# tzmhuang/OmniIsaacGymEnvs

Measured on AMD Instinct MI355X. Metric: env-steps/s (physics+obs+reward) Humanoid 4096 envs @1/2/4/8 MI355X, higher is better.
Workload: dtype f32

## Files before the change

include/mi_geom.h:

```cpp
#ifndef MI_GEOM_H
#define MI_GEOM_H

#include <math.h>

#if defined(__HIPCC__)
#define MI_GEOM_FN static inline __host__ __device__
#else
#define MI_GEOM_FN static inline
#endif

#if defined(__clang__)
#define MI_GEOM_NO_CONTRACT _Pragma("clang fp contract(off)")
#else
#define MI_GEOM_NO_CONTRACT
#endif

MI_GEOM_FN float mi_g_clamp01(float x) { return x < 0.0f ? 0.0f : (x > 1.0f ? 1.0f : x); }

MI_GEOM_FN void mi_segment_closest(const float* a0, const float* a1, const float* b0,
                                   const float* b1, float* ca, float* cb) {
    MI_GEOM_NO_CONTRACT
    float d1[3], d2[3], r[3];
    for (int k = 0; k < 3; ++k) { d1[k] = a1[k] - a0[k]; d2[k] = b1[k] - b0[k]; r[k] = a0[k] - b0[k]; }
    const float a = d1[0] * d1[0] + d1[1] * d1[1] + d1[2] * d1[2];
    const float e = d2[0] * d2[0] + d2[1] * d2[1] + d2[2] * d2[2];
    const float f = d2[0] * r[0] + d2[1] * r[1] + d2[2] * r[2];
    float s = 0.0f, t = 0.0f;
    if (a <= 1e-12f && e <= 1e-12f) {
        s = 0.0f; t = 0.0f;
    } else if (a <= 1e-12f) {
        s = 0.0f; t = mi_g_clamp01(f / e);
    } else {
        const float c = d1[0] * r[0] + d1[1] * r[1] + d1[2] * r[2];
        if (e <= 1e-12f) {
            t = 0.0f; s = mi_g_clamp01(-c / a);
        } else {
            const float b = d1[0] * d2[0] + d1[1] * d2[1] + d1[2] * d2[2];
            const float den = a * e - b * b;
            s = den > 1e-12f ? mi_g_clamp01((b * f - c * e) / den) : 0.0f;
            t = (b * s + f) / e;
            if (t < 0.0f) { t = 0.0f; s = mi_g_clamp01(-c / a); }
            else if (t > 1.0f) { t = 1.0f; s = mi_g_clamp01((b - c) / a); }
        }
    }
    for (int k = 0; k < 3; ++k) { ca[k] = a0[k] + d1[k] * s; cb[k] = b0[k] + d2[k] * t; }
}

MI_GEOM_FN void mi_contact_basis(const float* n, float* t1, float* t2) {
    MI_GEOM_NO_CONTRACT
    const float ax[3] = {n[0] < 0.57735f && n[0] > -0.57735f ? 1.0f : 0.0f,
                         n[0] < 0.57735f && n[0] > -0.57735f ? 0.0f : 1.0f, 0.0f};
    float c[3] = {n[1] * ax[2] - n[2] * ax[1], n[2] * ax[0] - n[0] * ax[2], n[0] * ax[1] - n[1] * ax[0]};
    const float cl = sqrtf(c[0] * c[0] + c[1] * c[1] + c[2] * c[2]);
    for (int k = 0; k < 3; ++k) t1[k] = c[k] / cl;
    t2[0] = n[1] * t1[2] - n[2] * t1[1];
    t2[1] = n[2] * t1[0] - n[0] * t1[2];
    t2[2] = n[0] * t1[1] - n[1] * t1[0];
}

MI_GEOM_FN float mi_pair_contact(const float* a0, const float* a1, float ra, const float* b0,
                                 const float* b1, float rb, float* pc, float* n) {
    MI_GEOM_NO_CONTRACT
    float ca[3], cb[3];
    mi_segment_closest(a0, a1, b0, b1, ca, cb);
    float d[3] = {ca[0] - cb[0], ca[1] - cb[1], ca[2] - cb[2]};
    const float dist = sqrtf(d[0] * d[0] + d[1] * d[1] + d[2] * d[2]);
    if (dist > 1e-9f) {
        for (int k = 0; k < 3; ++k) n[k] = d[k] / dist;
    } else {
        n[0] = 0.0f; n[1] = 0.0f; n[2] = 1.0f;
    }
    const float gap = dist - ra - rb;
    for (int k = 0; k < 3; ++k) pc[k] = cb[k] + n[k] * (rb + 0.5f * gap);
    return gap;
}

#endif
```

include/mi_sim.h:

```cpp
#ifndef MI_SIM_H
#define MI_SIM_H

#include <stdint.h>

#ifdef __cplusplus
extern "C" {
#endif

#define MI_ABI_VERSION 4

enum {
    MI_OK = 0,
    MI_E_NULL = -1,
    MI_E_SHAPE = -2,
    MI_E_HIP = -3,
    MI_E_MODEL = -4,
    MI_E_ARG = -5,
    MI_E_NODEV = -6,
    MI_E_STATE = -7
};

enum { MI_TASK_CARTPOLE = 0, MI_TASK_ANT = 1, MI_TASK_HUMANOID = 2 };

enum {
// ... 128 lines not shown
int mi_get_state_mirror(mi_sim* sim, void* stream);

int mi_sim_step(mi_sim* sim, int32_t substeps, void* stream);
int mi_sim_flush(mi_sim* sim, void* stream);

int mi_task_configure(mi_sim* sim, const mi_task_params* tp);
int mi_task_pre_step(mi_sim* sim, const float* actions , int64_t* reset_buf,
                     int64_t* progress_buf, float* potentials, float* prev_potentials,
                     float* actions_out , void* stream);
int mi_task_reset_idx(mi_sim* sim, const int64_t* env_ids, int32_t n, int64_t* reset_buf,
                      int64_t* progress_buf, float* potentials, float* prev_potentials,
                      void* stream);
int mi_task_post_step(mi_sim* sim, const float* actions , float* obs ,
                      float* rew , int64_t* reset_buf, int64_t* progress_buf,
                      float* potentials, float* prev_potentials, void* stream);
int mi_task_post_kernel(const mi_sim* sim, int32_t* kernel, int32_t* grid);
int mi_task_observations(mi_sim* sim, const float* actions , float* obs ,
                         float* potentials, float* prev_potentials, void* stream);
int mi_task_metrics(mi_sim* sim, const float* actions, const float* obs, float* rew,
                    const float* potentials, const float* prev_potentials, void* stream);
int mi_task_is_done(mi_sim* sim, const float* obs, int64_t* reset_buf, const int64_t* progress_buf,
                    void* stream);
int mi_env_step(mi_sim* sim, const float* actions , int32_t substeps,
                float* obs_out , float* obs_task ,
                float* rew , int64_t* reset_buf, int64_t* progress_buf,
                float* potentials, float* prev_potentials, float* actions_out ,
                float* rew_out , int64_t* reset_out , void* stream);
int mi_sim_time_launches(mi_sim* sim, int32_t every, int32_t capacity);
int mi_sim_launch_times(mi_sim* sim, float* ms_out, int32_t max_out, int32_t* n_out);

enum { MI_DR_OP_ADDITIVE = 0, MI_DR_OP_SCALING = 1 };
enum { MI_DR_DIST_GAUSSIAN = 0, MI_DR_DIST_UNIFORM = 1, MI_DR_DIST_LOGUNIFORM = 2 };
typedef struct mi_dr_noise {
    int32_t enabled;
    int32_t operation;
    int32_t distribution;
    int32_t frequency_interval;
    float params[2];
} mi_dr_noise;
typedef struct mi_dr_params {
    mi_dr_noise obs_on_reset, obs_on_interval, act_on_reset, act_on_interval;
} mi_dr_params;
int mi_task_set_dr(mi_sim* sim, const mi_dr_params* dr );
int mi_dr_apply_actions(mi_sim* sim, float* actions , const int64_t* reset_buf, void* stream);
int mi_dr_apply_observations(mi_sim* sim, float* obs , const int64_t* reset_buf,
                             void* stream);
int mi_get_dr_state(mi_sim* sim, uint32_t* out );

enum { MI_ENVP_GRAVITY = 0,
       MI_ENVP_FRICTION = 1,
       MI_ENVP_DAMPING = 2,
       MI_ENVP_ARMATURE = 3    };
int mi_set_env_params(mi_sim* sim, int32_t attr, const float* values ,
                      const int64_t* idx , int32_t n, void* stream);
int mi_get_env_params(mi_sim* sim, int32_t attr, float* out , void* stream);
int mi_sim_clear_env_params(mi_sim* sim);

enum { MI_DR_OP_DIRECT = 2 };
typedef struct mi_dr_phys_sched {
    int32_t enabled;
    int32_t operation;
    int32_t distribution;
    int32_t frequency_interval;
    const float* p0;
    const float* p1;
} mi_dr_phys_sched;
typedef struct mi_dr_phys_params {
    mi_dr_phys_sched on_reset[4], on_interval[4];
    int32_t min_frequency;
} mi_dr_phys_params;
int mi_sim_set_phys_dr(mi_sim* sim, const mi_dr_phys_params* dr );
int mi_dr_phys_step(mi_sim* sim, const int64_t* reset_buf , void* stream);
int mi_get_phys_dr_state(mi_sim* sim, uint32_t* out );

int mi_fill_uniform(mi_sim* sim, float* out , int32_t cols, uint64_t seed,
                    uint64_t step, float lo, float hi, void* stream);
int mi_get_reset_count(mi_sim* sim, uint32_t* out );
int mi_set_reset_count(mi_sim* sim, const uint32_t* in );
int mi_sim_pair_load(mi_sim* sim, int32_t* out , const int32_t* in ,
                     int32_t pairing);
int mi_sim_nan_count(mi_sim* sim, int64_t* count);
int mi_sim_kernel_path(const mi_sim* sim, int32_t* path, int32_t* topology, int32_t* lds_bytes);
int mi_sim_w_rows_lds(const mi_sim* sim, int32_t* rows);
int mi_abi_version(void);
const char* mi_build_id(void);
const char* mi_last_error(void);

#ifdef __cplusplus
}
#endif
#endif
```

omniisaacgymenvs_amd/csrc/mi_pair.hpp:

```cpp
#pragma once
#include "mi_wave.hpp"

#ifndef MI_PAIR_SOLVE_PD
#define MI_PAIR_SOLVE_PD 3
#endif
#ifndef MI_PRIO_C1
#define MI_PRIO_C1 12
#endif
#ifndef MI_PRIO_C2
#define MI_PRIO_C2 18
#endif
#ifndef MI_PRIO_C3
#define MI_PRIO_C3 27
#endif

namespace mi {

MI_D float pbc(float v, int k) {
    const float a = readlane(v, k), b = readlane(v, k + 32);
    return (pair_l64() & 32) ? b : a;
}
template <int K>
MI_D float pbcc(float v) {
    static_assert(K >= 0 && K < 32, "lane of the half");
// ... 200 lines not shown
    wave_sync();
    STAMP(0);
    for (int l = 1 + lane; l < L; l += 32) wave_link_local(mc, t, sm, l);
    wave_sync();
    for (int l = lane; l < L; l += 32) wave_link_forward<TP::kEnvP>(mc, nr, t, sm, l, p, ep);
    wave_sync();
    STAMP(1);
    float* aux = sm + t.s_X;
    {
        const pv4* recs = reinterpret_cast<const pv4*>(sm + t.s_F);
        for (int l = lane; l < L; l += 32) {
            pv4 a0 = recs[4 * l], a1 = recs[4 * l + 1], a2 = recs[4 * l + 2], a3 = recs[4 * l + 3];
            for (int di = mc.desc_start(l); di < mc.desc_start(l + 1); ++di) {
                const int d = mc.desc(di);
                a0 += recs[4 * d];
                a1 += recs[4 * d + 1];
                a2 += recs[4 * d + 2];
                a3 += recs[4 * d + 3];
            }
            pv4* o = reinterpret_cast<pv4*>(aux) + 4 * l;
            o[0] = a0; o[1] = a1; o[2] = a2; o[3] = a3;
        }
    }
    wave_sync();
    STAMP(2);
    phase_p3_bias_crba<Grp32, TP>(lane, i, D, nv, nr, dt, us, rhs, Mx, Ss, mc, t, st, aux, ep);
    wave_sync();
    STAMP(3);
    float Mc[TP::nvc];
    ct_load_columns<TP>(Mx, lane, Mc);
    const float dvec = ct_ltdl_pair<TP>(lane, Mc);
    STAMP(5);
    {
        const int dj = lane < nr ? lane : __builtin_popcount(mc.mask(lane < nv ? lane - nr + 1 : 0)) - 1;
        ct_publish_factor<TP>(lane, dj, Mc, dvec, sm + t.s_L);
    }
    STAMP(4);
    int ncon = 0;
    {
        const float rpz = sm[t.s_rp + 2];
        for (int c0 = 0; c0 < t.npts; c0 += 32) {
            const int c = c0 + lane;
            bool act = false;
            float pc[3] = {0, 0, 0}, bn = 0.0f;
            int l = 0;
            if (c < t.npts) {
                l = (int)mc.pf(MP_LINK, c);
                const float pl[3] = {mc.pf(MP_X, c), mc.pf(MP_X + 1, c), mc.pf(MP_X + 2, c)};
                float R[9], x[3];
#pragma unroll
                for (int q = 0; q < 9; ++q) R[q] = sm[t.s_R + 9 * l + q];
                m3_vec(R, pl, x);
#pragma unroll
                for (int q = 0; q < 3; ++q) x[q] += sm[t.s_o + 3 * l + q];
                const float rr = mc.pf(MP_RAD, c);
                const float gap = rpz + x[2] - rr;
                act = gap < p.contact_offset;
                pc[0] = x[0]; pc[1] = x[1]; pc[2] = x[2] - rr;
                const float d = gap - p.rest_offset;
                bn = p.tgs ? d : row_bias(p, d, dt, true);
            }
            const unsigned mask = hballot(act);
            if (act) {
                const int ci = ncon + __popc(mask & lanemask_lt(lane));
#pragma unroll
                for (int q = 0; q < 3; ++q) sm[t.s_cp + 3 * ci + q] = pc[q];
                sm[t.s_cl + ci] = (float)l;
                sm[t.s_cl2 + ci] = -1.0f;
#pragma unroll
                for (int tt = 0; tt < 3; ++tt) {
                    const int r = 3 * ci + tt;
                    sm[t.s_rl + r] = (float)l;
                    sm[t.s_rb + r] = tt == 0 ? bn : 0.0f;
                }
            }
            ncon += __popc(mask);
        }
    }
    if constexpr (TP::kSelf) {
        if (t.self_on) {
            float* seg = sm + t.s_seg;
            float* bnd = seg + 8 * t.ngeoms;
            const float* geo = mcb + t.mc_geo;
            const int2* gpr = reinterpret_cast<const int2*>(t.g_pairs);
            int2 gpf[5];
#pragma unroll
            for (int q = 0; q < 5; ++q) {
                const int pi = 32 * q + lane;
                gpf[q] = pi < t.npairs ? gpr[pi] : make_int2(0, 0);
            }
            for (int g = lane; g < t.ngeoms; g += 32) {
                const float* A = geo + 8 * g;
                const int l = (int)A[0];
                float R[9], a0[3], a1[3];
#pragma unroll
                for (int q = 0; q < 9; ++q) R[q] = sm[t.s_R + 9 * l + q];
                m3_vec(R, A + 1, a0); m3_vec(R, A + 4, a1);
#pragma unroll
                for (int q = 0; q < 3; ++q) {
                    seg[8 * g + q] = a0[q] + sm[t.s_o + 3 * l + q];
                    seg[8 * g + 3 + q] = a1[q] + sm[t.s_o + 3 * l + q];
                }
                seg[8 * g + 6] = A[7];
                seg[8 * g + 7] = (float)l;
                float e2 = 0.0f;
#pragma unroll
                for (int q = 0; q < 3; ++q) {
                    bnd[4 * g + q] = sm[t.s_o + 3 * l + q] + 0.5f * (a0[q] + a1[q]);
                    e2 += (a1[q] - a0[q]) * (a1[q] - a0[q]);
                }
                bnd[4 * g + 3] = 0.5f * sqrtf(e2) + A[7];
            }
            wave_sync();
            int* surv = reinterpret_cast<int*>(sm + t.s_surv);
            int nsv = 0;
            const float slack = p.contact_offset + 1e-3f;
            auto broad = [&](int pb, int2 gpq, bool pref) {
                const int pi = pb + lane;
                bool keep = false;
                int2 gp = make_int2(0, 0);
                if (pi < t.npairs) {
                    gp = pref ? gpq : gpr[pi];
                    const float4 A = *reinterpret_cast<const float4*>(bnd + 4 * gp.x);
                    const float4 B = *reinterpret_cast<const float4*>(bnd + 4 * gp.y);
                    const float cx = A.x - B.x, cy = A.y - B.y, cz = A.z - B.z;
                    const float reach = A.w + B.w + slack;
                    keep = cx * cx + cy * cy + cz * cz < reach * reach;
                }
                const unsigned mask = hballot(keep);
                if (keep) surv[nsv + __popc(mask & lanemask_lt(lane))] = gp.x | (gp.y << 16);
                nsv += __popc(mask);
            };
            sfor<0, 5>([&](auto Q) { if (32 * (int)Q < t.npairs) broad(32 * (int)Q, gpf[Q], true); });
            for (int pb = 160; pb < t.npairs; pb += 32) broad(pb, make_int2(0, 0), false);
            wave_sync();
            int budget = (MI_MAX_ROWS - 3 * ncon - t.nlimc) / 3;
            const int nsv_max = pmax(nsv);
            for (int sb = 0; sb < nsv_max; sb += 32) {
                const int sidx = sb + lane;
                bool act = false;
                float pc[3], n[3], bn = 0.0f;
                int la = 0, lb = 0;
                if (sidx < nsv && budget > 0) {
                    const int pk = surv[sidx];
                    const float* A = seg + 8 * (pk & 0xffff);
                    const float* B = seg + 8 * (pk >> 16);
                    la = (int)A[7]; lb = (int)B[7];
                    const float gap = mi_pair_contact(A, A + 3, A[6], B, B + 3, B[6], pc, n);
                    act = gap < p.contact_offset;
                    const float d = gap - p.rest_offset;
                    bn = p.tgs ? d : row_bias(p, d, dt, true);
                }
                const unsigned mask = hballot(act);
                const int rank = __popc(mask & lanemask_lt(lane));
                if (act && rank < budget) {
                    const int ci = ncon + rank;
#pragma unroll
                    for (int q = 0; q < 3; ++q) { sm[t.s_cp + 3 * ci + q] = pc[q]; sm[t.s_cn + 3 * ci + q] = n[q]; }
                    sm[t.s_cl + ci] = (float)la;
                    sm[t.s_cl2 + ci] = (float)lb;
#pragma unroll
                    for (int tt = 0; tt < 3; ++tt) {
                        const int r = 3 * ci + tt;
                        sm[t.s_rl + r] = (float)la;
                        sm[t.s_rb + r] = tt == 0 ? bn : 0.0f;
                    }
                }
                const int took = budget > 0 ? min(__popc(mask), budget) : 0;
                ncon += took;
                budget -= took;
            }
        }
    }
    const int nc = 3 * ncon;
    {
        const int cr = pmax(nc);
        if (cr > MI_PRIO_C3 && prio < 3) { __builtin_amdgcn_s_setprio(3); prio = 3; }
        else if (cr > MI_PRIO_C2 && prio < 2) { __builtin_amdgcn_s_setprio(2); prio = 2; }
        else if (cr > MI_PRIO_C1 && prio < 1) { __builtin_amdgcn_s_setprio(1); prio = 1; }
    }
    wave_sync();
    STAMP(6);
    constexpr bool kSpec = TP::D >= MI_PAIR_LIM_SPEC_MIN_D;
    unsigned cmask = 0u, nmask = 0u;
    if constexpr (kSpec) {
        bool cand = false, near = false;
        if (lane < D) {
            const float lo = mc.lf(MC_LO, lane + 1), hi = mc.lf(MC_HI, lane + 1);
            const float qj = sm[t.s_q + lane], qp = qj + dt * us[nr + lane];
            const float mg = MI_PAIR_LIM_NEAR;
            cand = lo < hi;
            near = cand && (qj < lo + mg || qp < lo + mg || qj > hi - mg || qp > hi - mg);
        }
        cmask = hballot(cand);
        nmask = hballot(near);
    }
    const unsigned fmask = cmask & ~nmask;
    const int nN = __popc(nmask);
    const int nspec = kSpec ? min(__popc(cmask), 31 - (nc & 31)) : t.nlimc;
    int total = nc + 1 + nspec;
    int total_max = pmax(total);
    unsigned rem = 0u;
    int nrows = nc;
    unsigned limact = 0u;
    auto limit_rows = [&](const auto& res, bool here, bool rhs_lane) {
        constexpr int NR = sizeof(res) / sizeof(res[0]);
        if (rhs_lane) {
#pragma unroll
            for (int c = 0; c < NR; ++c)
                if (c < TP::nv) us[c] = us[c] + dt * res[c];
        }
        wave_sync();
        bool act = false;
        float bl = 0.0f, sg = 0.0f;
        if (here && lane < D) {
            const int l = lane + 1, k = nr + lane;
            const float lo = mc.lf(MC_LO, l), hi = mc.lf(MC_HI, l);
            if (lo < hi) {
                const float qj = sm[t.s_q + lane];
                const float qp = qj + dt * us[k];
                float d = 0.0f;
                if (qj < lo || qp < lo) { d = qj - lo; sg = 1.0f; act = true; }
                else if (qj > hi || qp > hi) { d = hi - qj; sg = -1.0f; act = true; }
                bl = p.tgs ? d : row_bias(p, d, dt, true);
            }
        }
        const unsigned lb = hballot(act);
        if (here) limact = lb;
        if (act) {
            const int rl = nc + __popc(limact & lanemask_lt(lane));
// ... 795 lines not shown
```

omniisaacgymenvs_amd/csrc/mi_sim.hip:

```cpp
#include <hip/hip_runtime.h>
#include <hip/hip_ext.h>

#include <cmath>
#include <cstdarg>
#include <cstdio>
#include <cstring>
#include <string>
#include <vector>
#include <algorithm>

#include "mi_artic.hpp"
#include "mi_device.hpp"
#include "mi_task.hpp"
#include "mi_wave.hpp"
#include "mi_pair.hpp"
#include "mi_link.hpp"
#include "mi_dyn.hpp"
#include "mi_msolve.hpp"
#include "mi_idyn.hpp"

using namespace mi;

static thread_local std::string g_err;

// ... 1143 lines not shown
    if (s->wave) {
        const char* tsel = getenv("MI_SIM_TOPO");
        s->topo = (tsel && std::string(tsel) == "runtime") ? 0 : match_topology(cx.md, self_on);
    }
    return MI_OK;
}

static int create_tree_tables(mi_sim* s, CreateCtx& cx) {
    const mi_model_desc* md = cx.md;
    const DevModel& m = s->dm;
    WaveTabs& t = s->wt;
    const int L = m.L;
    const std::vector<int>& dof_parent = cx.dof_parent;
    std::vector<int> depth(L, 0);
    int maxd = 0;
    for (int l = 1; l < L; ++l) { depth[l] = depth[md->parent[l]] + 1; maxd = std::max(maxd, depth[l]); }
    t.nlev = maxd + 1;
    std::vector<int> lev_start(t.nlev + 1, 0), lev_links;
    for (int d = 0; d < t.nlev; ++d) {
        lev_start[d] = (int)lev_links.size();
        for (int l = 0; l < L; ++l) if (depth[l] == d) lev_links.push_back(l);
    }
    lev_start[t.nlev] = (int)lev_links.size();
    std::vector<int> child_start(L + 1, 0), child_list;
    for (int l = 0; l < L; ++l) {
        child_start[l] = (int)child_list.size();
        for (int c = l + 1; c < L; ++c) if (md->parent[c] == l) child_list.push_back(c);
    }
    child_start[L] = (int)child_list.size();
    std::vector<int>&desc_start = cx.desc_start, &desc_list = cx.desc_list;
    desc_start.assign(L + 1, 0);
    for (int l = 0; l < L; ++l) {
        desc_start[l] = (int)desc_list.size();
        for (int c = l + 1; c < L; ++c) {
            int x = md->parent[c];
            while (x > l) x = md->parent[x];
            if (x == l) desc_list.push_back(c);
        }
    }
    desc_start[L] = (int)desc_list.size();
    if (desc_list.empty()) desc_list.push_back(0);
    std::vector<int>& anc_start = cx.anc_start;
    anc_start.assign(m.nv + 1, 0);
    std::vector<int> anc_list;
    int na_max = 0;
    for (int k = 0; k < m.nv; ++k) {
        anc_start[k] = (int)anc_list.size();
        for (int j = dof_parent[k]; j >= 0; j = dof_parent[j]) anc_list.push_back(j);
        na_max = std::max(na_max, (int)anc_list.size() - anc_start[k]);
    }
    anc_start[m.nv] = (int)anc_list.size();
    std::vector<unsigned long long>& link_mask = cx.link_mask;
    link_mask.assign(L, 0ull);
    for (int l = 0; l < L; ++l) {
        unsigned long long msk = 0ull;
        for (int k = 0; k < m.nr; ++k) msk |= 1ull << k;
        for (int x = l; x > 0; x = md->parent[x]) msk |= 1ull << (m.nr + x - 1);
        link_mask[l] = msk;
    }
    std::vector<unsigned char> tri_p, tri_q;
    for (int q = 0; q < na_max; ++q)
        for (int p2 = 0; p2 <= q; ++p2) { tri_p.push_back((unsigned char)p2); tri_q.push_back((unsigned char)q); }
    if (tri_p.empty()) { tri_p.push_back(0); tri_q.push_back(0); }
    if (child_list.empty()) child_list.push_back(0);
    if (anc_list.empty()) anc_list.push_back(0);
    UPW(lev_start, lev_start); UPW(lev_links, lev_links); UPW(child_start, child_start);
    UPW(child_list, child_list); UPW(anc_start, anc_start); UPW(anc_list, anc_list);
    UPW(desc_start, desc_start); UPW(desc_list, desc_list);
    std::vector<int>&chain_start = cx.chain_start, &chain_list = cx.chain_list;
    chain_start.assign(L + 1, 0);
    for (int l = 0; l < L; ++l) {
        chain_start[l] = (int)chain_list.size();
        std::vector<int> up;
        for (int x = l; x > 0; x = md->parent[x]) up.push_back(x);
        chain_list.insert(chain_list.end(), up.rbegin(), up.rend());
    }
    chain_start[L] = (int)chain_list.size();
    if (chain_list.empty()) chain_list.push_back(0);
    UPW(chain_start, chain_start); UPW(chain_list, chain_list);
    UPW(link_mask, link_mask); UPW(tri_p, tri_p); UPW(tri_q, tri_q);
    return MI_OK;
}

static int create_constant_block(mi_sim* s, const CreateCtx& cx) {
    const mi_model_desc* md = cx.md;
    WaveTabs& t = s->wt;
    const int L = s->dm.L;
    const bool self_on = cx.self_on;
    const std::vector<int>&pt_geom = cx.pt_geom, &pt_end = cx.pt_end, &chain_start = cx.chain_start,
                          &chain_list = cx.chain_list, &desc_start = cx.desc_start, &desc_list = cx.desc_list;
    const std::vector<unsigned long long>& link_mask = cx.link_mask;
    {
        const int np = (int)pt_geom.size(), ns = md->num_sensors;
        std::vector<float> mcb((size_t)MC_NLINKF * L, 0.0f);
        for (int l = 0; l < L; ++l) {
            auto put = [&](int f, float v) { mcb[(size_t)f * L + l] = v; };
            for (int c = 0; c < 3; ++c) {
                put(MC_POS + c, md->pos[3 * l + c]); put(MC_AXIS + c, md->axis[3 * l + c]);
                put(MC_COM + c, md->com[3 * l + c]);
            }
            for (int c = 0; c < 4; ++c) put(MC_QUAT + c, md->quat[4 * l + c]);
            for (int c = 0; c < 6; ++c) put(MC_INER + c, md->inertia[6 * l + c]);
            put(MC_JTYPE, (float)md->jtype[l]); put(MC_MASS, md->mass[l]);
            put(MC_ARM, md->armature[l]); put(MC_DAMP, md->damping[l]);
            put(MC_LO, md->lower[l]); put(MC_HI, md->upper[l]);
            const unsigned lo32 = (unsigned)(link_mask[l] & 0xffffffffull);
            float mf; std::memcpy(&mf, &lo32, 4); put(MC_MASK, mf);
        }
        auto pad4 = [&]() { while (mcb.size() % 4) mcb.push_back(0.0f); };
        pad4();
        t.mc_pts = (int)mcb.size();
        mcb.resize(mcb.size() + (size_t)MP_NF * np, 0.0f);
        for (int c = 0; c < np; ++c) {
            const int g = pt_geom[c];
            const float* pg = pt_end[c] ? md->geom_p1 + 3 * g : md->geom_p0 + 3 * g;
            mcb[t.mc_pts + (size_t)MP_LINK * np + c] = (float)md->geom_link[g];
            for (int q = 0; q < 3; ++q) mcb[t.mc_pts + (size_t)(MP_X + q) * np + c] = pg[q];
            mcb[t.mc_pts + (size_t)MP_RAD * np + c] = md->geom_radius[g];
        }
        pad4();
        t.mc_sens = (int)mcb.size();
        mcb.resize(mcb.size() + (size_t)MS_NF * ns, 0.0f);
        for (int c = 0; c < ns; ++c) {
            mcb[t.mc_sens + (size_t)MS_LINK * ns + c] = (float)md->sensor_link[c];
            for (int q = 0; q < 3; ++q)
                mcb[t.mc_sens + (size_t)(MS_X + q) * ns + c] = md->sensor_pos[3 * c + q];
        }
        auto put_ints = [&](const std::vector<int>& v) {
            pad4();
            const int at = (int)mcb.size();
            for (int x : v) { float f; std::memcpy(&f, &x, 4); mcb.push_back(f); }
            return at;
        };
        t.mc_chs = put_ints(chain_start); t.mc_chl = put_ints(chain_list);
        t.mc_dss = put_ints(desc_start); t.mc_dsl = put_ints(desc_list);
        std::vector<int> lim;
        for (int l = 1; l < L; ++l)
            if (md->lower[l] < md->upper[l]) lim.push_back(l - 1);
        t.nlimc = (int)lim.size();
        if (lim.empty()) lim.push_back(0);
        t.mc_lim = put_ints(lim);
        std::vector<float> geo((size_t)8 * std::max(1, md->num_geoms), 0.0f);
        for (int g = 0; g < md->num_geoms; ++g) {
            geo[8 * g] = (float)md->geom_link[g];
            for (int q = 0; q < 3; ++q) {
                geo[8 * g + 1 + q] = md->geom_p0[3 * g + q];
                geo[8 * g + 4 + q] = md->geom_p1[3 * g + q];
            }
            geo[8 * g + 7] = md->geom_radius[g];
        }
        std::vector<int> prs(md->pairs ? md->pairs : nullptr,
                             md->pairs ? md->pairs + 2 * md->num_pairs : nullptr);
        if (prs.empty()) prs.assign(2, 0);
        t.mc_geo = t.mc_pairs = -1;
        if (self_on) {
            pad4();
            t.mc_geo = (int)mcb.size();
            mcb.insert(mcb.end(), geo.begin(), geo.begin() + 8 * md->num_geoms);
        }
        pad4();
        t.mc_len = (int)mcb.size();
        t.npts = np; t.nsens = ns;
        UPW(g_mc, mcb);
        UPW(g_geo, geo); UPW(g_pairs, prs);
    }
    return MI_OK;
}

struct LdsLayout {
    const DevModel& m;
    WaveTabs& t;
    bool ct, self_on;
    int L, lr, env_budget, R, C, waves, lam_rows;
    int so = 0, ro = 0, span0 = 0, span1 = 0;
    bool overlay = false;
    static int al4(int x) { return (x + 3) & ~3; }
    int take(int n) { const int at = so; so += al4(n); return at; }
    int take_r(int n) { const int at = ro; ro += al4(n); return at; }
    void paired();
    void one_per_wave();
};

void LdsLayout::paired() {
    t.s_mc = take(t.mc_len);
    t.s_R = take(9 * L); t.s_o = take(3 * L); t.s_S = take(6 * m.nv);
    t.s_D = take(4); t.s_r = take(WNV); t.s_us = take(WNV); t.s_q = take(WNV); t.s_rp = take(8);
    t.s_xs = take(4);
    t.s_L = take(lr + m.nv);
    t.j_rows_lds = 0;
    t.s_J = take(4);
    t.s_lam = take(4);
    span0 = so;
    t.s_F = take(16 * L); t.s_Ic = take(4); t.s_M = take(m.nv * m.nv); t.s_X = take(16 * L);
    span1 = so;
    overlay = true;
    ro = span0;
    t.s_cp = take_r(3 * C); t.s_cl = take_r(C); t.s_cl2 = take_r(C); t.s_cn = take_r(3 * C);
    t.s_rl = take_r(R); t.s_rb = take_r(R); t.s_rk = -1; t.s_ad = take_r(R);
    t.s_lsg = take_r(WNV);
    t.s_W = ro;
    int w = std::min(64, (t.s_R + env_budget - ro) / m.nv);
    while (w > 0 && ro + al4(w * m.nv) > t.s_R + env_budget) --w;
    w &= ~3;
    t.w_rows_lds = t.w_rows_a = std::max(0, w);
    const char* spe = getenv("MI_SENS_PAR");
    t.sens_par = (!spe || atoi(spe) != 0) && 6 * m.S * (C + 1) <= t.w_rows_lds * m.nv ? 1 : 0;
    t.s_W2 = 0;
    so = std::max(span1, ro + al4(t.w_rows_lds * m.nv));
}

void LdsLayout::one_per_wave() {
    t.s_mc = take(t.mc_len);
    t.s_R = take(9 * L); t.s_o = take(3 * L); t.s_S = take(6 * m.nv);
    span0 = so;
    t.s_F = take(16 * L);
    t.s_Ic = take(4);
    t.s_M = take(m.nv * m.nv);
    t.s_X = take(16 * L);
    span1 = so;
    t.s_D = take(ct ? 4 : WNV); t.s_r = take(WNV); t.s_us = take(WNV);
    t.s_q = take(WNV); t.s_rp = take(8);
    const int rows_len = 8 * al4(C) + 4 * al4(R) + WNV;
    overlay = ct && rows_len <= span1 - span0;
    ro = overlay ? span0 : so;
    t.s_cp = take_r(3 * C); t.s_cl = take_r(C); t.s_cl2 = take_r(C); t.s_cn = take_r(3 * C);
    t.s_rl = take_r(R);
    t.s_rb = take_r(R); t.s_rk = take_r(R); t.s_ad = take_r(R); t.s_lsg = take_r(WNV);
    if (!overlay) so = ro;
    t.s_xs = take(ct ? 4 : WNV * 64);
    t.s_L = take(ct ? lr + m.nv : 4);
    t.j_rows_lds = ct ? std::min(waves >= 4 ? lam_rows : 48, m.max_rows) : 0;
    t.s_J = take(t.j_rows_lds > 0 ? t.j_rows_lds * m.nv : 4);
    t.s_lam = take(4);
    t.s_W = ro;
    t.w_rows_lds = overlay ? std::min(64, (span1 - ro) / m.nv) : 0;
    t.w_rows_a = t.w_rows_lds;
    t.s_W2 = 0;
    {
        const int want = std::min(64, m.max_rows);
        const int lds_budget_floats = t.s_R + env_budget;
        int fit = want;
        while (fit > 0 && so + al4(fit * m.nv) > lds_budget_floats) --fit;
        if (ct && t.w_rows_lds < fit && (fit == want || !self_on)) {
            t.s_W = take(fit * m.nv);
            t.w_rows_lds = t.w_rows_a = fit;
        } else if (ct && self_on && t.w_rows_lds < want) {
            const int extra = std::min(want - t.w_rows_lds, (lds_budget_floats - so - 3) / m.nv);
            if (extra > 0) {
                t.s_W2 = take(extra * m.nv);
                t.w_rows_lds += extra;
            }
        }
    }
}

static int create_lds_layout(mi_sim* s, const CreateCtx& cx) {
    const mi_model_desc* md = cx.md;
    const DevModel& m = s->dm;
    WaveTabs& t = s->wt;
    const int L = m.L, N = s->N;
    const bool self_on = cx.self_on;
    const std::vector<int>& anc_start = cx.anc_start;
    auto al4 = [](int x) { return LdsLayout::al4(x); };
    const bool ct = s->topo != 0;
    int waves = 2, lam_rows = 0;
    bool pair_ok = false;
    with_topo(s->topo, s->sp.tgs != 0, [&](auto T) {
        waves = decltype(T)::kWaves; lam_rows = decltype(T)::kLamRows;
        pair_ok = has_pair<decltype(T)>();
    });
    const char* pe = getenv("MI_WAVE_PAIR");
    const bool pair_want = pe ? atoi(pe) != 0 : true;
    s->pair = ct && pair_ok && N % 2 == 0 && pair_want;
    const int envs_cu = s->pair ? 16 : 4 * std::max(1, waves);
    t.envs_per_wg = s->pair ? 16 : (ct && waves >= 4 ? 4 : 1);
    if (const char* e = getenv("MI_WAVE_ENVS"); e && !s->pair) t.envs_per_wg = std::max(1, std::min(4, atoi(e)));
    const int E = t.envs_per_wg;
    const int env_budget = ((163840 / (int)sizeof(float)) / std::max(1, envs_cu / E) - al4(t.mc_len)) / E;
    const int R = m.max_rows;
    t.self_on = self_on ? 1 : 0;
    t.npairs = self_on ? md->num_pairs : 0;
    t.ncmax = std::min(m.npts + t.npairs, MI_MAX_ROWS / 3);
    const int C = t.ncmax;
    int lr = 0;
    for (int k = 0; k < m.nv; ++k) lr += (anc_start[k + 1] - anc_start[k] + 3) & ~3;
    LdsLayout lay{m, t, ct, self_on, L, lr, env_budget, R, C, waves, lam_rows};
    if (s->pair) lay.paired();
    else lay.one_per_wave();
    const int so = lay.so, ro = lay.ro, span0 = lay.span0, span1 = lay.span1;
    const bool overlay = lay.overlay;
    t.s_total = so;
    t.s_env = t.s_R;
    t.env_stride = so - t.s_env;
    if (!s->pair) {
        const int offs[] = {t.s_mc, t.s_R, t.s_o, t.s_S, t.s_F, t.s_Ic, t.s_M, t.s_X,
                            t.s_D, t.s_r, t.s_us, t.s_q, t.s_rp, t.s_xs, t.s_L, t.s_J,
                            t.s_lam, t.s_total};
        for (size_t c = 1; c < sizeof(offs) / sizeof(offs[0]); ++c)
            if (offs[c] <= offs[c - 1]) return fail(MI_E_STATE, "wave LDS layout: region %zu overlaps", c);
        const bool rows_ok = overlay ? (t.s_cp == span0 && ro <= span1)
                                     : (t.s_cp > t.s_rp && ro <= t.s_xs);
        if (!rows_ok) return fail(MI_E_STATE, "wave LDS layout: row data misplaced");
    }
    t.max_rows = m.max_rows;
    t.g_row_stride = (size_t)m.max_rows * WNV;
    t.ngeoms = md->num_geoms;
    t.s_seg = -1; t.s_surv = -1;
    if (overlay && self_on && al4(12 * md->num_geoms) + al4(md->num_pairs) <= span1 - ro) {
        t.s_seg = ro;
        t.s_surv = ro + al4(12 * md->num_geoms);
    }
    s->lds_bytes = (size_t)(so + (t.envs_per_wg - 1) * t.env_stride) * sizeof(float);
    if (getenv("MI_SIM_DEBUG"))
        fprintf(stderr, "[mi_sim] wave layout: pair=%d envs/wg=%d lds/wg=%zu B env_stride=%d floats "
                        "mc=%d w_rows_lds=%d (a %d) j_rows_lds=%d s_seg=%d max_rows=%d ncmax=%d\n",
                (int)s->pair, t.envs_per_wg, s->lds_bytes, t.env_stride, t.mc_len, t.w_rows_lds,
                t.w_rows_a, t.j_rows_lds, t.s_seg, m.max_rows, t.ncmax);
    if (s->pair && ((self_on && t.s_seg < 0) || s->lds_bytes > 163840))
        return fail(MI_E_STATE, "paired wave layout does not fit (%zu B of LDS per workgroup)",
                            s->lds_bytes);
    if (s->pair && t.w_rows_lds < lam_rows)
        return fail(MI_E_STATE, "paired wave layout: %d LDS W rows < %d Delassus rows",
                            t.w_rows_lds, lam_rows);
    return MI_OK;
}

static int create_params(mi_sim* s, const mi_sim_params* prm) {
    s->sp.dt = prm->dt;
    for (int k = 0; k < 3; ++k) s->sp.g[k] = prm->gravity[k];
    if (prm->solver_type != MI_SOLVER_PGS && prm->solver_type != MI_SOLVER_TGS)
        return fail(MI_E_ARG, "solver_type %d: this build implements 0 (PGS) and 1 (TGS)",
                            prm->solver_type);
    if (prm->solver_iterations < 1 || prm->solver_iterations > 64 || prm->velocity_iterations < 0 ||
        prm->velocity_iterations > 64)
        return fail(MI_E_ARG, "solver iterations %d / velocity iterations %d out of range",
                            prm->solver_iterations, prm->velocity_iterations);
    s->sp.iters = prm->solver_iterations;
    s->sp.tgs = prm->solver_type == MI_SOLVER_TGS ? 1 : 0;
    s->sp.viters = s->sp.tgs ? prm->velocity_iterations : 0;
    s->sp.h = s->sp.tgs ? prm->dt / (float)prm->solver_iterations : prm->dt;
    s->sp.contact_offset = prm->contact_offset;
    s->sp.rest_offset = prm->rest_offset;
    s->sp.friction = prm->friction;
    s->sp.max_depen = prm->max_depenetration_velocity;
    s->sp.erp = prm->erp;
    s->sp.max_angvel = prm->max_angular_velocity;
    s->sp.ang_damp = prm->angular_damping;
    if (!(prm->angular_damping >= 0.0f)) return fail(MI_E_ARG, "angular_damping must be >= 0");
    return MI_OK;
}

static int create_state(mi_sim* s, int64_t off, uint64_t seed, const float* env_origins) {
    const DevModel& m = s->dm;
    const int N = s->N;
    int rc = 0;
    DevState& st = s->ds;
// ... 1140 lines not shown
```

omniisaacgymenvs_amd/csrc/mi_wave.hpp:

```cpp
#pragma once
#include "mi_artic.hpp"
#include "mi_device.hpp"
#include "mi_topo_gen.hpp"
#include "../../include/mi_geom.h"

namespace mi {

constexpr int WNV = 32;

__device__ __forceinline__ int wave_lane() { return (int)(threadIdx.x & 63u); }
__device__ __forceinline__ void wave_sync() {
    __builtin_amdgcn_fence(__ATOMIC_RELEASE, "wavefront");
    __builtin_amdgcn_wave_barrier();
    __builtin_amdgcn_fence(__ATOMIC_ACQUIRE, "wavefront");
}

#ifdef MI_STAMPS
#define MI_STAMP_SLOTS 16384
#define MI_STAMP_ENV (blockIdx.x * (blockDim.x >> 6) + (threadIdx.x >> 6))
__device__ unsigned long long g_phase[MI_STAMP_SLOTS][32];
#define STAMP_BEGIN()                                                                     \
    unsigned long long stamp_t_;                                                          \
    do {                                                                                  \
        __builtin_amdgcn_sched_barrier(0);                                                \
        asm volatile("s_memtime %0\n\ts_waitcnt lgkmcnt(0)" : "=s"(stamp_t_)::"memory");  \
        __builtin_amdgcn_sched_barrier(0);                                                \
    } while (0)
#define STAMP(id)                                                                         \
    do {                                                                                  \
        __builtin_amdgcn_sched_barrier(0);                                                \
        unsigned long long t_;                                                            \
        asm volatile("s_memtime %0\n\ts_waitcnt lgkmcnt(0)" : "=s"(t_)::"memory");         \
        if ((threadIdx.x & 63) == 0) g_phase[MI_STAMP_ENV % MI_STAMP_SLOTS][id] += t_ - stamp_t_;  \
        stamp_t_ = t_;                                                                    \
        __builtin_amdgcn_sched_barrier(0);                                                \
    } while (0)
#define STAMP_END()                                                                       \
    do {                                                                                  \
        if ((threadIdx.x & 63) == 0) g_phase[MI_STAMP_ENV % MI_STAMP_SLOTS][31] += 1ull;           \
    } while (0)
#define STAT(id, v)                                                                       \
    do {                                                                                  \
        if ((threadIdx.x & 63) == 0) g_phase[MI_STAMP_ENV % MI_STAMP_SLOTS][id] += (unsigned long long)(v); \
    } while (0)
#define STAMP_RESET()                                                                     \
    do {                                                                                  \
        __builtin_amdgcn_sched_barrier(0);                                                \
        asm volatile("s_memtime %0\n\ts_waitcnt lgkmcnt(0)" : "=s"(stamp_t_)::"memory");  \
        __builtin_amdgcn_sched_barrier(0);                                                \
    } while (0)
#else
#define STAT(id, v) do { } while (0)
#define STAMP_RESET() do { } while (0)
#define STAMP_BEGIN() do { } while (0)
#define STAMP(id) do { } while (0)
#define STAMP_END() do { } while (0)
#endif

struct WaveTabs {
    int nlev;
    const int* lev_start;
    const int* lev_links;
    const int* child_start;
    const int* child_list;
    const int* chain_start;
    const int* chain_list;
    const int* desc_start;
    const int* desc_list;
    const int* anc_start;
    const int* anc_list;
    const unsigned long long* link_mask;
    const unsigned char* tri_p;
    const unsigned char* tri_q;
    int s_mc, s_R, s_o, s_S, s_F, s_Ic, s_M, s_X, s_D, s_r, s_us, s_q, s_rp, s_cp, s_cl,
        s_rl, s_lsg, s_rb, s_rk, s_ad, s_xs, s_L, s_total;
    int max_rows;
    size_t g_row_stride;
    int s_W, w_rows_lds;
    int s_W2, w_rows_a;
    int envs_per_wg, s_env, env_stride;
    int s_J, j_rows_lds;
    const float* g_mc;
    int mc_len, mc_pts, mc_sens, mc_chs, mc_chl, mc_dss, mc_dsl, mc_lim;
    int mc_geo, mc_pairs;
    int npts, nsens;
    int nlimc;
    int self_on, npairs, ncmax;
    const float* g_geo;
    const int* g_pairs;
    int s_cl2, s_cn;
    int s_seg, s_surv;
    int ngeoms;
    int s_lam;
    int sens_par;
    float* g_wa;
};

enum McField {
    MC_POS = 0, MC_QUAT = 3, MC_AXIS = 7, MC_JTYPE = 10, MC_MASS = 11, MC_COM = 12,
    MC_INER = 15, MC_ARM = 21, MC_DAMP = 22, MC_LO = 23, MC_HI = 24, MC_MASK = 25,
    MC_NLINKF = 26
};
enum McPoint { MP_LINK = 0, MP_X = 1, MP_RAD = 4, MP_NF = 5 };
enum McSensor { MS_LINK = 0, MS_X = 1, MS_NF = 4 };

struct MC {
    const float* b;
    const int* bi;
    int L, np, ns;
    const WaveTabs* t;
    MI_D float lf(int f, int l) const { return b[f * L + l]; }
    MI_D void lf3(int f, int l, float* o) const { o[0] = lf(f, l); o[1] = lf(f + 1, l); o[2] = lf(f + 2, l); }
    MI_D int jtype(int l) const { return (int)lf(MC_JTYPE, l); }
    MI_D unsigned mask(int l) const { return (unsigned)bi[MC_MASK * L + l]; }
    MI_D float pf(int f, int c) const { return b[t->mc_pts + f * np + c]; }
    MI_D float sf(int f, int s) const { return b[t->mc_sens + f * ns + s]; }
    MI_D int chain_start(int l) const { return bi[t->mc_chs + l]; }
    MI_D int chain(int j) const { return bi[t->mc_chl + j]; }
    MI_D int desc_start(int l) const { return bi[t->mc_dss + l]; }
    MI_D int desc(int j) const { return bi[t->mc_dsl + j]; }
    MI_D int lim(int j) const { return bi[t->mc_lim + j]; }
};

template <bool SELF>
MI_D void contact_dirs(const float* sm, const WaveTabs& t, int ci, float (&d)[9]) {
    if (!SELF || sm[t.s_cl2 + ci] < 0.0f) {
#pragma unroll
        for (int k = 0; k < 9; ++k) d[k] = (k == 2 || k == 3 || k == 7) ? 1.0f : 0.0f;
    } else {
        d[0] = sm[t.s_cn + 3 * ci]; d[1] = sm[t.s_cn + 3 * ci + 1]; d[2] = sm[t.s_cn + 3 * ci + 2];
        mi_contact_basis(d, d + 3, d + 6);
    }
}

template <bool SELF>
MI_D void contact_row_f(const float* sm, const WaveTabs& t, int r, float (&f)[6]) {
    const int ci = r / 3, tt = r - 3 * ci;
    const float pc[3] = {sm[t.s_cp + 3 * ci], sm[t.s_cp + 3 * ci + 1], sm[t.s_cp + 3 * ci + 2]};
    float d[9];
    contact_dirs<SELF>(sm, t, ci, d);
    const float dir[3] = {d[3 * tt], d[3 * tt + 1], d[3 * tt + 2]};
    cross3(pc, dir, f);
    f[3] = dir[0]; f[4] = dir[1]; f[5] = dir[2];
}

MI_D MC make_mc(const WaveTabs& t, const float* mcb, int L) {
    MC c;
    c.b = mcb;
    c.bi = (const int*)mcb;
    c.L = L; c.np = t.npts; c.ns = t.nsens;
    c.t = &t;
    return c;
}

MI_D float wave_sum(float v) {
#pragma unroll
    for (int o = 32; o >= 1; o >>= 1) v += __shfl_xor(v, o, 64);
    return v;
}
template <bool SEG2>
MI_D float* w_row(const WaveTabs& t, float* sm, int r, int nv) {
    if constexpr (!SEG2) return sm + t.s_W + r * nv;
    return sm + (r < t.w_rows_a ? t.s_W + r * nv : t.s_W2 + (r - t.w_rows_a) * nv);
}

MI_D float readlane(float v, int l) {
    return __int_as_float(__builtin_amdgcn_readlane(__float_as_int(v), l));
// ... 1265 lines not shown
```

omniisaacgymenvs_amd/native.py:

```python
from __future__ import annotations

import ctypes as C
import os
from typing import Optional

import numpy as np

_HERE = os.path.dirname(os.path.abspath(__file__))
LIB_PATH = os.environ.get("MI_SIM_LIB", os.path.join(_HERE, "libmi_sim.so"))

MI_OK = 0
MI_TASK_CARTPOLE, MI_TASK_ANT, MI_TASK_HUMANOID = 0, 1, 2
MI_DYN_ARTICULATION, MI_DYN_CARTPOLE = 0, 1
MI_SOLVER_PGS, MI_SOLVER_TGS = 0, 1
MI_JOINT_HINGE, MI_JOINT_SLIDE = 0, 1
MI_GEOM_SPHERE, MI_GEOM_CAPSULE = 0, 1

_f32p = C.POINTER(C.c_float)
_i32p = C.POINTER(C.c_int32)
_i64p = C.POINTER(C.c_int64)


class MiModelDesc(C.Structure):
    _fields_ = [
# ... 60 lines not shown
                ("frequency_interval", C.c_int32), ("p0", _f32p), ("p1", _f32p)]


class MiDrPhysParams(C.Structure):
    _fields_ = [("on_reset", MiDrPhysSched * 4), ("on_interval", MiDrPhysSched * 4),
                ("min_frequency", C.c_int32)]


def fptr(a: Optional[np.ndarray]):
    return None if a is None else a.ctypes.data_as(_f32p)


def iptr(a: Optional[np.ndarray]):
    return None if a is None else a.ctypes.data_as(_i32p)


class NativeUnavailable(RuntimeError):
    """libmi_sim.so could not be used: not built, failed to load, or no GPU."""


_LIB = None

_SIGS = {
    "mi_sim_create": (C.c_int, [C.POINTER(MiModelDesc), C.POINTER(MiSimParams), C.c_int32,
                                C.c_int64, C.c_int32, C.c_void_p, C.c_uint64, C.POINTER(C.c_void_p)]),
    "mi_sim_destroy": (C.c_int, [C.c_void_p]),
    "mi_sim_info": (C.c_int, [C.c_void_p, _i32p, _i32p, _i32p, _i32p, C.c_void_p]),
    "mi_get_root_state": (C.c_int, [C.c_void_p] + [C.c_void_p] * 4),
    "mi_get_dof_state": (C.c_int, [C.c_void_p] + [C.c_void_p] * 3),
    "mi_get_sensor_wrench": (C.c_int, [C.c_void_p, C.c_void_p, C.c_void_p]),
    "mi_get_link_state": (C.c_int, [C.c_void_p, _i32p, _f32p, C.c_int32, C.c_void_p, C.c_void_p, C.c_void_p,
                                    C.c_void_p]),
    "mi_get_link_jacobian": (C.c_int, [C.c_void_p, _i32p, _f32p, C.c_int32, C.c_void_p, C.c_void_p]),
    "mi_get_dynamics": (C.c_int, [C.c_void_p] + [C.c_void_p] * 4),
    "mi_solve_mass": (C.c_int, [C.c_void_p, C.c_int32, C.c_void_p, C.c_int32, C.c_void_p, C.c_void_p]),
    "mi_get_forward_dynamics": (C.c_int, [C.c_void_p, C.c_int32, C.c_void_p, C.c_void_p, C.c_void_p]),
    "mi_get_link_task_inertia": (C.c_int, [C.c_void_p, C.c_int32, _i32p, _f32p, C.c_int32, C.c_void_p, C.c_void_p,
                                           C.c_void_p]),
    "mi_get_inverse_dynamics": (C.c_int, [C.c_void_p, C.c_int32, C.c_void_p, C.c_void_p, C.c_void_p, C.c_void_p]),
    "mi_get_link_acceleration": (C.c_int, [C.c_void_p, _i32p, _f32p, C.c_int32, C.c_void_p, C.c_void_p, C.c_void_p]),
    "mi_get_momentum": (C.c_int, [C.c_void_p] + [C.c_void_p] * 5),
    "mi_set_dof_efforts": (C.c_int, [C.c_void_p, C.c_void_p, C.c_void_p, C.c_int32, C.c_void_p]),
    "mi_set_dof_state": (C.c_int, [C.c_void_p, C.c_void_p, C.c_void_p, C.c_void_p, C.c_int32,
                                   C.c_void_p]),
    "mi_set_root_state": (C.c_int, [C.c_void_p, C.c_void_p, C.c_void_p, C.c_void_p, C.c_void_p,
                                    C.c_int32, C.c_void_p]),
    "mi_set_dof_state_i32": (C.c_int, [C.c_void_p, C.c_void_p, C.c_void_p, C.c_void_p, C.c_int32,
                                       C.c_void_p]),
    "mi_set_root_state_i32": (C.c_int, [C.c_void_p, C.c_void_p, C.c_void_p, C.c_void_p, C.c_void_p,
                                        C.c_int32, C.c_void_p]),
    "mi_sim_set_mirror": (C.c_int, [C.c_void_p] + [C.c_void_p] * 6),
    "mi_get_state_mirror": (C.c_int, [C.c_void_p, C.c_void_p]),
    "mi_sim_step": (C.c_int, [C.c_void_p, C.c_int32, C.c_void_p]),
    "mi_sim_flush": (C.c_int, [C.c_void_p, C.c_void_p]),
    "mi_task_configure": (C.c_int, [C.c_void_p, C.POINTER(MiTaskParams)]),
    "mi_task_pre_step": (C.c_int, [C.c_void_p] + [C.c_void_p] * 7),
    "mi_task_reset_idx": (C.c_int, [C.c_void_p, C.c_void_p, C.c_int32] + [C.c_void_p] * 5),
    "mi_task_post_step": (C.c_int, [C.c_void_p] + [C.c_void_p] * 8),
    "mi_task_post_kernel": (C.c_int, [C.c_void_p, _i32p, _i32p]),
    "mi_task_observations": (C.c_int, [C.c_void_p] + [C.c_void_p] * 5),
    "mi_task_metrics": (C.c_int, [C.c_void_p] + [C.c_void_p] * 6),
    "mi_task_is_done": (C.c_int, [C.c_void_p] + [C.c_void_p] * 4),
    "mi_env_step": (C.c_int, [C.c_void_p, C.c_void_p, C.c_int32] + [C.c_void_p] * 11),
    "mi_sim_time_launches": (C.c_int, [C.c_void_p, C.c_int32, C.c_int32]),
    "mi_sim_launch_times": (C.c_int, [C.c_void_p, C.c_void_p, C.c_int32, _i32p]),
    "mi_task_set_dr": (C.c_int, [C.c_void_p, C.POINTER(MiDrParams)]),
    "mi_dr_apply_actions": (C.c_int, [C.c_void_p, C.c_void_p, C.c_void_p, C.c_void_p]),
    "mi_dr_apply_observations": (C.c_int, [C.c_void_p, C.c_void_p, C.c_void_p, C.c_void_p]),
    "mi_get_dr_state": (C.c_int, [C.c_void_p, C.c_void_p]),
    "mi_set_env_params": (C.c_int, [C.c_void_p, C.c_int32, C.c_void_p, C.c_void_p, C.c_int32, C.c_void_p]),
    "mi_get_env_params": (C.c_int, [C.c_void_p, C.c_int32, C.c_void_p, C.c_void_p]),
    "mi_sim_clear_env_params": (C.c_int, [C.c_void_p]),
    "mi_sim_set_phys_dr": (C.c_int, [C.c_void_p, C.POINTER(MiDrPhysParams)]),
    "mi_dr_phys_step": (C.c_int, [C.c_void_p, C.c_void_p, C.c_void_p]),
    "mi_get_phys_dr_state": (C.c_int, [C.c_void_p, C.c_void_p]),
    "mi_fill_uniform": (C.c_int, [C.c_void_p, C.c_void_p, C.c_int32, C.c_uint64, C.c_uint64,
                                  C.c_float, C.c_float, C.c_void_p]),
    "mi_get_reset_count": (C.c_int, [C.c_void_p, C.c_void_p]),
    "mi_set_reset_count": (C.c_int, [C.c_void_p, C.c_void_p]),
    "mi_sim_pair_load": (C.c_int, [C.c_void_p, C.c_void_p, C.c_void_p, C.c_int32]),
    "mi_sim_nan_count": (C.c_int, [C.c_void_p, _i64p]),
    "mi_sim_kernel_path": (C.c_int, [C.c_void_p, _i32p, _i32p, _i32p]),
    "mi_sim_w_rows_lds": (C.c_int, [C.c_void_p, _i32p]),
    "mi_abi_version": (C.c_int, []),
    "mi_build_id": (C.c_char_p, []),
    "mi_last_error": (C.c_char_p, []),
}

EXPORTED_SYMBOLS = tuple(_SIGS)


def load_library(path: str = LIB_PATH) -> C.CDLL:
    if not os.path.exists(path):
        raise NativeUnavailable(
            f"{path} is missing: build it with `python -c 'import __graft_entry__ as g; g.build()'`")
    try:
        lib = C.CDLL(path)
    except OSError as e:
        raise NativeUnavailable(f"failed to load {path}: {e}") from e
    lenient = "MI_SIM_LIB" in os.environ and path == LIB_PATH
    for name, (res, args) in _SIGS.items():
        try:
            fn = getattr(lib, name)
        except AttributeError:
            if lenient and name == "mi_build_id":
                continue
            raise
        fn.restype = res
        fn.argtypes = args
    return lib


def lib() -> C.CDLL:
    global _LIB
    if _LIB is None:
        _LIB = load_library()
    return _LIB


def check(rc: int, what: str = "") -> None:
    if rc != MI_OK:
        msg = lib().mi_last_error()
        raise RuntimeError(f"{what or 'mi_sim'} failed ({rc}): {msg.decode() if msg else ''}")


def ptr(t) -> Optional[int]:
    if t is None:
        return None
    return t.data_ptr()
```

Baseline: 40.66 million.

## Precompute self-collision bound radii and pack pair table into LDS constant block

On the pair-wave path, when the model is small enough, each geom's bounding radius is computed once on the host and stored in the constant block. The self-collision pair list is stored there too as packed 8-bit indices, and the broadphase reads both from LDS instead of recomputing the radius and loading int2 pairs from global memory. The J/lambda stub LDS slots are aliased when the tables are present, and the link index is stored as raw int bits instead of a float conversion. This removes per-step global loads and a sqrt per geom, in exchange for extra LDS use in the constant block and the loss of the register-prefetched pair loop.

```diff
diff --git a/include/mi_geom.h b/include/mi_geom.h
--- a/include/mi_geom.h
+++ b/include/mi_geom.h
@@ -75,4 +75,10 @@
     return gap;
 }
 
+MI_GEOM_FN float mi_geom_bound_radius(const float* p0, const float* p1, float radius) {
+    MI_GEOM_NO_CONTRACT
+    const float d[3] = {p1[0] - p0[0], p1[1] - p0[1], p1[2] - p0[2]};
+    return 0.5f * sqrtf(d[0] * d[0] + d[1] * d[1] + d[2] * d[2]) + radius;
+}
+
 #endif
diff --git a/include/mi_sim.h b/include/mi_sim.h
--- a/include/mi_sim.h
+++ b/include/mi_sim.h
@@ -234,6 +234,7 @@
 int mi_sim_nan_count(mi_sim* sim, int64_t* count);
 int mi_sim_kernel_path(const mi_sim* sim, int32_t* path, int32_t* topology, int32_t* lds_bytes);
 int mi_sim_w_rows_lds(const mi_sim* sim, int32_t* rows);
+int mi_model_bound_radii(const mi_model_desc* model, float* out );
 int mi_abi_version(void);
 const char* mi_build_id(void);
 const char* mi_last_error(void);
diff --git a/omniisaacgymenvs_amd/csrc/mi_pair.hpp b/omniisaacgymenvs_amd/csrc/mi_pair.hpp
--- a/omniisaacgymenvs_amd/csrc/mi_pair.hpp
+++ b/omniisaacgymenvs_amd/csrc/mi_pair.hpp
@@ -306,13 +306,7 @@
             float* seg = sm + t.s_seg;
             float* bnd = seg + 8 * t.ngeoms;
             const float* geo = mcb + t.mc_geo;
-            const int2* gpr = reinterpret_cast<const int2*>(t.g_pairs);
-            int2 gpf[5];
-#pragma unroll
-            for (int q = 0; q < 5; ++q) {
-                const int pi = 32 * q + lane;
-                gpf[q] = pi < t.npairs ? gpr[pi] : make_int2(0, 0);
-            }
+            const bool tabs = t.mc_pairs >= 0;
             for (int g = lane; g < t.ngeoms; g += 32) {
                 const float* A = geo + 8 * g;
                 const int l = (int)A[0];
@@ -326,37 +320,52 @@
                     seg[8 * g + 3 + q] = a1[q] + sm[t.s_o + 3 * l + q];
                 }
                 seg[8 * g + 6] = A[7];
-                seg[8 * g + 7] = (float)l;
-                float e2 = 0.0f;
-#pragma unroll
-                for (int q = 0; q < 3; ++q) {
+                seg[8 * g + 7] = __int_as_float(l);
+#pragma unroll
+                for (int q = 0; q < 3; ++q)
                     bnd[4 * g + q] = sm[t.s_o + 3 * l + q] + 0.5f * (a0[q] + a1[q]);
-                    e2 += (a1[q] - a0[q]) * (a1[q] - a0[q]);
-                }
-                bnd[4 * g + 3] = 0.5f * sqrtf(e2) + A[7];
+                if (tabs) {
+                    bnd[4 * g + 3] = mcb[t.mc_brad + g];
+                } else {
+                    float e2 = 0.0f;
+#pragma unroll
+                    for (int q = 0; q < 3; ++q) e2 += (a1[q] - a0[q]) * (a1[q] - a0[q]);
+                    bnd[4 * g + 3] = 0.5f * sqrtf(e2) + A[7];
+                }
             }
             wave_sync();
             int* surv = reinterpret_cast<int*>(sm + t.s_surv);
             int nsv = 0;
             const float slack = p.contact_offset + 1e-3f;
-            auto broad = [&](int pb, int2 gpq, bool pref) {
-                const int pi = pb + lane;
-                bool keep = false;
-                int2 gp = make_int2(0, 0);
-                if (pi < t.npairs) {
-                    gp = pref ? gpq : gpr[pi];
-                    const float4 A = *reinterpret_cast<const float4*>(bnd + 4 * gp.x);
-                    const float4 B = *reinterpret_cast<const float4*>(bnd + 4 * gp.y);
-                    const float cx = A.x - B.x, cy = A.y - B.y, cz = A.z - B.z;
-                    const float reach = A.w + B.w + slack;
-                    keep = cx * cx + cy * cy + cz * cz < reach * reach;
-                }
-                const unsigned mask = hballot(keep);
-                if (keep) surv[nsv + __popc(mask & lanemask_lt(lane))] = gp.x | (gp.y << 16);
-                nsv += __popc(mask);
+            auto broad = [&](auto kTab) {
+                typedef const unsigned short __attribute__((address_space(3)))* lds_cu16;
+                const lds_cu16 ptab = (lds_cu16)(mcb + (kTab ? t.mc_pairs : 0));
+                const int2* gpr = reinterpret_cast<const int2*>(t.g_pairs);
+                for (int pb = 0; pb < t.npairs; pb += 32) {
+                    const int pi = pb + lane;
+                    bool keep = false;
+                    int ga = 0, gb = 0;
+                    if (pi < t.npairs) {
+                        if constexpr (decltype(kTab)::value) {
+                            const int pk = ptab[pi];
+                            ga = pk & 0xff; gb = pk >> 8;
+                        } else {
+                            const int2 gp = gpr[pi];
+                            ga = gp.x; gb = gp.y;
+                        }
+                        const float4 A = *reinterpret_cast<const float4*>(bnd + 4 * ga);
+                        const float4 B = *reinterpret_cast<const float4*>(bnd + 4 * gb);
+                        const float cx = A.x - B.x, cy = A.y - B.y, cz = A.z - B.z;
+                        const float reach = A.w + B.w + slack;
+                        keep = cx * cx + cy * cy + cz * cz < reach * reach;
+                    }
+                    const unsigned mask = hballot(keep);
+                    if (keep) surv[nsv + __popc(mask & lanemask_lt(lane))] = ga | (gb << 16);
+                    nsv += __popc(mask);
+                }
             };
-            sfor<0, 5>([&](auto Q) { if (32 * (int)Q < t.npairs) broad(32 * (int)Q, gpf[Q], true); });
-            for (int pb = 160; pb < t.npairs; pb += 32) broad(pb, make_int2(0, 0), false);
+            if (tabs) broad(std::true_type{});
+            else broad(std::false_type{});
             wave_sync();
             int budget = (MI_MAX_ROWS - 3 * ncon - t.nlimc) / 3;
             const int nsv_max = pmax(nsv);
@@ -369,7 +378,7 @@
                     const int pk = surv[sidx];
                     const float* A = seg + 8 * (pk & 0xffff);
                     const float* B = seg + 8 * (pk >> 16);
-                    la = (int)A[7]; lb = (int)B[7];
+                    la = __float_as_int(A[7]); lb = __float_as_int(B[7]);
                     const float gap = mi_pair_contact(A, A + 3, A[6], B, B + 3, B[6], pc, n);
                     act = gap < p.contact_offset;
                     const float d = gap - p.rest_offset;
diff --git a/omniisaacgymenvs_amd/csrc/mi_sim.hip b/omniisaacgymenvs_amd/csrc/mi_sim.hip
--- a/omniisaacgymenvs_amd/csrc/mi_sim.hip
+++ b/omniisaacgymenvs_amd/csrc/mi_sim.hip
@@ -1249,6 +1249,22 @@
     return MI_OK;
 }
 
+static bool pair_path_selected(const mi_sim* s) {
+    bool pair_ok = false;
+    with_topo(s->topo, s->sp.tgs != 0, [&](auto T) { pair_ok = has_pair<decltype(T)>(); });
+    const char* pe = getenv("MI_WAVE_PAIR");
+    return s->topo != 0 && pair_ok && s->N % 2 == 0 && (pe ? atoi(pe) != 0 : true);
+}
+
+int mi_model_bound_radii(const mi_model_desc* md, float* out) {
+    if (!md || !out) return fail(MI_E_NULL, "mi_model_bound_radii: null argument");
+    if (md->num_geoms > 0 && (!md->geom_p0 || !md->geom_p1 || !md->geom_radius))
+        return fail(MI_E_NULL, "mi_model_bound_radii: geom arrays must not be null");
+    for (int g = 0; g < md->num_geoms; ++g)
+        out[g] = mi_geom_bound_radius(md->geom_p0 + 3 * g, md->geom_p1 + 3 * g, md->geom_radius[g]);
+    return MI_OK;
+}
+
 static int create_constant_block(mi_sim* s, const CreateCtx& cx) {
     const mi_model_desc* md = cx.md;
     WaveTabs& t = s->wt;
@@ -1319,11 +1335,29 @@
         std::vector<int> prs(md->pairs ? md->pairs : nullptr,
                              md->pairs ? md->pairs + 2 * md->num_pairs : nullptr);
         if (prs.empty()) prs.assign(2, 0);
-        t.mc_geo = t.mc_pairs = -1;
+        t.mc_geo = t.mc_brad = t.mc_pairs = -1;
         if (self_on) {
             pad4();
             t.mc_geo = (int)mcb.size();
             mcb.insert(mcb.end(), geo.begin(), geo.begin() + 8 * md->num_geoms);
+            const int G = md->num_geoms, P = md->num_pairs;
+            const int need = ((G + 3) & ~3) + (((P + 1) / 2 + 3) & ~3);
+            if (pair_path_selected(s) && G <= 256 && need <= kPairSelfTabs) {
+                pad4();
+                t.mc_brad = (int)mcb.size();
+                std::vector<float> br((size_t)G);
+                mi_model_bound_radii(md, br.data());
+                mcb.insert(mcb.end(), br.begin(), br.end());
+                pad4();
+                t.mc_pairs = (int)mcb.size();
+                for (int q = 0; q < P; q += 2) {
+                    unsigned w = 0;
+                    for (int h = 0; h < 2 && q + h < P; ++h)
+                        w |= (unsigned)(md->pairs[2 * (q + h)] | md->pairs[2 * (q + h) + 1] << 8) << (16 * h);
+                    float f; std::memcpy(&f, &w, 4); mcb.push_back(f);
+                }
+                mcb.resize((size_t)t.mc_brad + kPairSelfTabs, 0.0f);
+            }
         }
         pad4();
         t.mc_len = (int)mcb.size();
@@ -1355,8 +1389,9 @@
     t.s_xs = take(4);
     t.s_L = take(lr + m.nv);
     t.j_rows_lds = 0;
-    t.s_J = take(4);
-    t.s_lam = take(4);
+    const bool stubs = t.mc_pairs < 0;
+    t.s_J = stubs ? take(4) : so;
+    t.s_lam = stubs ? take(4) : so;
     span0 = so;
     t.s_F = take(16 * L); t.s_Ic = take(4); t.s_M = take(m.nv * m.nv); t.s_X = take(16 * L);
     span1 = so;
@@ -1431,14 +1466,10 @@
     auto al4 = [](int x) { return LdsLayout::al4(x); };
     const bool ct = s->topo != 0;
     int waves = 2, lam_rows = 0;
-    bool pair_ok = false;
     with_topo(s->topo, s->sp.tgs != 0, [&](auto T) {
         waves = decltype(T)::kWaves; lam_rows = decltype(T)::kLamRows;
-        pair_ok = has_pair<decltype(T)>();
     });
-    const char* pe = getenv("MI_WAVE_PAIR");
-    const bool pair_want = pe ? atoi(pe) != 0 : true;
-    s->pair = ct && pair_ok && N % 2 == 0 && pair_want;
+    s->pair = pair_path_selected(s);
     const int envs_cu = s->pair ? 16 : 4 * std::max(1, waves);
     t.envs_per_wg = s->pair ? 16 : (ct && waves >= 4 ? 4 : 1);
     if (const char* e = getenv("MI_WAVE_ENVS"); e && !s->pair) t.envs_per_wg = std::max(1, std::min(4, atoi(e)));
diff --git a/omniisaacgymenvs_amd/csrc/mi_wave.hpp b/omniisaacgymenvs_amd/csrc/mi_wave.hpp
--- a/omniisaacgymenvs_amd/csrc/mi_wave.hpp
+++ b/omniisaacgymenvs_amd/csrc/mi_wave.hpp
@@ -57,6 +57,8 @@
 #define STAMP_END() do { } while (0)
 #endif
 
+constexpr int kPairSelfTabs = 16 * 8;
+
 struct WaveTabs {
     int nlev;
     const int* lev_start;
@@ -82,7 +84,8 @@
     int s_J, j_rows_lds;
     const float* g_mc;
     int mc_len, mc_pts, mc_sens, mc_chs, mc_chl, mc_dss, mc_dsl, mc_lim;
-    int mc_geo, mc_pairs;
+    int mc_geo;
+    int mc_brad, mc_pairs;
     int npts, nsens;
     int nlimc;
     int self_on, npairs, ncmax;
diff --git a/omniisaacgymenvs_amd/native.py b/omniisaacgymenvs_amd/native.py
--- a/omniisaacgymenvs_amd/native.py
+++ b/omniisaacgymenvs_amd/native.py
@@ -166,6 +166,7 @@
     "mi_sim_nan_count": (C.c_int, [C.c_void_p, _i64p]),
     "mi_sim_kernel_path": (C.c_int, [C.c_void_p, _i32p, _i32p, _i32p]),
     "mi_sim_w_rows_lds": (C.c_int, [C.c_void_p, _i32p]),
+    "mi_model_bound_radii": (C.c_int, [C.POINTER(MiModelDesc), _f32p]),
     "mi_abi_version": (C.c_int, []),
     "mi_build_id": (C.c_char_p, []),
     "mi_last_error": (C.c_char_p, []),
@@ -187,7 +188,7 @@
         try:
             fn = getattr(lib, name)
         except AttributeError:
-            if lenient and name == "mi_build_id":
+            if lenient and name in ("mi_build_id", "mi_model_bound_radii"):
                 continue
             raise
         fn.restype = res
```

Result: no change. 40.54 million (-0.3%).
